# nishitbohra/RoViT-KAN-Interpretable-Vision-Transformer-for-Rose-Disease-Severity-Estimation

Measured on AMD Instinct MI355X. Metric: images/sec fwd+bwd, DeiT-Tiny+KAN 224^2, batch 256 per GPU, higher is better.
Workload: dtype bf16; 1 GPU; full RoViT-KAN (DeiT-Tiny + KAN + 3 heads) stage 4, train mode, batch 256/GPU, 224x224x3 randn images, random-init weights; step=fwd + JointLoss + bwd + grad all-reduce + clip_grad_norm(1.0) + AdamW, global_batch=256, parallelism=dp1, grad_buckets=2, rccl_world=0

## Files before the change

rovit-kan-interpretable-vision-transformer-for-rose-disease-severity-estimation_amd/csrc/gemm.hip:

```cpp
#include <cstdlib>
#include <type_traits>
#include "common.h"

#ifdef ROVIT_DEV
#define GEMM_DBG(g, bit) ((g).dbg & (bit))
#define GEMM_SET_DBG(g, v) (g).dbg = (v)
#else
#define GEMM_DBG(g, bit) (false)
#define GEMM_SET_DBG(g, v) ((void)0)
#endif

namespace {

inline bool set_max_lds(const void* fn, size_t bytes) { return rovit_set_max_lds(fn, bytes); }

constexpr int BK = 64;
constexpr int LDS_STRIDE = BK + 16;

enum { EPI_BF16 = 0, EPI_GELU = 1, EPI_RESID = 2, EPI_MUL = 3, EPI_PATCH = 4, EPI_RESID_LN = 5, EPI_LNBWD = 6,
       EPI_PATCH_IMG = 7 };

struct GemmArgs {
  const bf16* A; int lda;
  const bf16* W; int ldw;
// ... 777 lines not shown
        f32x4 o;
#pragma unroll
        for (int r = 0; r < 4; ++r) o[r] = dac[i][j][r] * gelu_grad((float)(bf16)pre[i][j][r]);
        const int row = i * 16 + l15;
        const int ch = 2 * (JT * wave + j) + (lg >> 1);
        const int phys = (ch & ~7) | ((ch & 7) ^ (row & 7));
        *(bf16x4*)(Cs + row * K + phys * 8 + 4 * (lg & 1)) = pack4(o);
      }
    barrier_lds();
    const int mbase = (tile0 + t) * BM;
#pragma unroll
    for (int q = 0; q < SMAX; ++q) {
      const int c = tid + q * NT;
      const int row = c / 24, ch = c - row * 24;
      const int m = mbase + row;
      if (m < g.M) {
        const int phys = (ch & ~7) | ((ch & 7) ^ (row & 7));
        *(bf16x8*)(g.out + (size_t)m * g.ldo + n0 + ch * 8) = *(const bf16x8*)(Cs + row * K + phys * 8);
      }
    }
    asm volatile("s_waitcnt lgkmcnt(0)" ::: "memory");
  }
}

template <int BM, int NW>
int launch_mlp_bwd(const MlpBwdArgs& g, hipStream_t st) {
  const int tiles_m = (g.M + BM - 1) / BM;
  int pmax = g_cu_budget * (768 / (NW * 64)) / g.n_tiles;
  pmax = pmax < 8 ? 8 : pmax / 8 * 8;
  const int tpw = (tiles_m + pmax - 1) / pmax;
  int P = (tiles_m + tpw - 1) / tpw;
  P = (P + 7) / 8 * 8;
  const size_t lds = (size_t)6 * BM * 192 * sizeof(bf16);
  ROVIT_CHECK_ARG(set_max_lds((const void*)mlp_bwd_dma_kernel<BM, NW>, lds), ROVIT_ERR_LAUNCH, "gemm_mlp_bwd: cannot raise the LDS limit");
  hipLaunchKernelGGL((mlp_bwd_dma_kernel<BM, NW>), dim3(P * g.n_tiles), dim3(NW * 64), lds, st, g, tpw, tiles_m);
  ROVIT_CHECK_LAUNCH("mlp_bwd_dma_kernel");
  return ROVIT_OK;
}

typedef unsigned int u32x2_t __attribute__((ext_vector_type(2)));

template <int KT, int EPI>
__global__ __launch_bounds__(768, 1) void gemm_kdma_kernel(const GemmArgs g, int tiles_per_wg, int n_tiles_m) {
  constexpr int K = 32 * KT, BM = 32, NT = 768;
  constexpr int CPRW = K / 8;
  constexpr int SLOT = BM * K;
  constexpr int PIECES = BM * CPRW / NT;
  constexpr int NSTORE = (EPI == EPI_RESID_LN) ? 7 : 6;
  constexpr int CSTR = 192 + 8;
  static_assert(BM * CPRW % NT == 0, "tile must split into whole DMA pieces");
  extern __shared__ __attribute__((aligned(16))) bf16 lds[];

  const int p = blockIdx.x;
  const int tile0 = p * tiles_per_wg;
  int ntile = n_tiles_m - tile0;
  ntile = ntile > tiles_per_wg ? tiles_per_wg : ntile;
  if (ntile <= 0) return;

  const int tid = threadIdx.x, lane = tid & 63, wave = tid >> 6;
  const int l15 = lane & 15, lg = lane >> 4;
  const bool row_wave = wave < 8;

  unsigned pk[PIECES];
#pragma unroll
  for (int i = 0; i < PIECES; ++i) {
    const int c = 64 * (wave + 12 * i) + lane;
    const int r = c / CPRW, x = c - r * CPRW;
    pk[i] = ((unsigned)r << 16) | (unsigned)(((x & ~7) | ((x & 7) ^ (r & 7))) * 8);
  }
  auto dma = [&](int tile, int slot) {
    const int row0 = tile * BM;
#pragma unroll
    for (int i = 0; i < PIECES; ++i) {
      unsigned q = pk[i];
      asm volatile("" : "+v"(q));
      int gr = row0 + (int)(q >> 16);
      gr = gr < g.M ? gr : g.M - 1;
      const bf16* src = g.A + ((unsigned)gr * (unsigned)g.lda + (q & 0xffffu));
      __builtin_amdgcn_global_load_lds((const __attribute__((address_space(1))) void*)src,
                                       (__attribute__((address_space(3))) void*)(lds + slot * SLOT + (wave + 12 * i) * 512), 16, 0, 0);
    }
  };
  dma(tile0, 0);
  if (ntile > 1) dma(tile0 + 1, 1);
  if (ntile > 2) dma(tile0 + 2, 2);

  bf16x8 wf[KT];
#pragma unroll
  for (int ks = 0; ks < KT; ++ks) wf[ks] = *(const bf16x8*)(g.W + (size_t)(16 * wave + l15) * g.ldw + ks * 32 + lg * 8);
  f32x4 bias4 = {0.f, 0.f, 0.f, 0.f};
  if (g.bias) {
    const float4 bb = *(const float4*)(g.bias + 16 * wave + 4 * lg);
    bias4 = (f32x4){bb.x, bb.y, bb.z, bb.w};
  }
  const int prow = tid >> 4, pc = tid & 15;
  wait_vmcnt<0>();

  for (int t = 0; t < ntile; ++t) {
    const int slot = t % 3;
    if (t >= 1) {
      if (t + 2 < ntile) { if (row_wave) wait_vmcnt<PIECES + NSTORE>(); else wait_vmcnt<PIECES>(); }
      else wait_vmcnt<0>();
    }
    __builtin_amdgcn_s_barrier();
    const int m = (tile0 + t) * BM + prow;
    const bool live = row_wave && m < g.M;
    const int mc = m < g.M ? m : g.M - 1;
    f32x4 xo0, xo1, xo2;
    u32x2_t hx0, hx1, hx2;
    float rr = 0.f;
    const unsigned xoff = (unsigned)mc * (unsigned)g.ldx + 4u * pc;
    float* xrow = g.xres + xoff;
    constexpr bool PREFETCH = KT <= 18;
    u32x2_t pv0, pv1, pv2;
    auto load_inputs = [&]() {
      if (EPI == EPI_LNBWD && g.xprev) {
        const bf16* prow_p = g.xprev + ((unsigned)mc * 192u + 4u * pc);
        pv0 = *(const u32x2_t*)prow_p; pv1 = *(const u32x2_t*)(prow_p + 64); pv2 = *(const u32x2_t*)(prow_p + 128);
      } else {
        xo0 = *(const f32x4*)xrow; xo1 = *(const f32x4*)(xrow + 64); xo2 = *(const f32x4*)(xrow + 128);
      }
      if (EPI == EPI_LNBWD) {
        const bf16* hrow = g.mul + ((unsigned)mc * (unsigned)g.ldm + 4u * pc);
        hx0 = *(const u32x2_t*)hrow; hx1 = *(const u32x2_t*)(hrow + 64); hx2 = *(const u32x2_t*)(hrow + 128);
        rr = g.pos[mc];
      }
    };
    if (PREFETCH && row_wave) load_inputs();
    const bool dma_now = t >= 1 && t + 2 < ntile;
    if (dma_now) dma(tile0 + t + 2, (t + 2) % 3);

    f32x4 acc[2] = {bias4, bias4};
    const bf16* Ac = lds + slot * SLOT;
#pragma unroll
    for (int ks = 0; ks < KT; ++ks) {
      const int lc = ks * 4 + lg;
#pragma unroll
      for (int i = 0; i < 2; ++i) {
        const int row = i * 16 + l15;
        const bf16x8 af = *(const bf16x8*)(Ac + row * K + ((lc & ~7) | ((lc & 7) ^ (row & 7))) * 8);
        acc[i] = mfma16(wf[ks], af, acc[i]);
      }
    }
    barrier_lds();
    bf16* Cs = lds + slot * SLOT;
#pragma unroll
    for (int i = 0; i < 2; ++i) *(bf16x4*)(Cs + (i * 16 + l15) * CSTR + 16 * wave + 4 * lg) = pack4(acc[i]);
    barrier_lds();
    if (row_wave) {
      if (!PREFETCH) load_inputs();
      float v[12];
#pragma unroll
      for (int i = 0; i < 3; ++i) {
        const bf16x4 tv = *(const bf16x4*)(Cs + prow * CSTR + 64 * i + 4 * pc);
#pragma unroll
        for (int e = 0; e < 4; ++e) v[4 * i + e] = (float)tv[e];
      }
      f32x4 xs[3] = {xo0, xo1, xo2};
      if (EPI == EPI_LNBWD && g.xprev) {
        const u32x2_t pvs[3] = {pv0, pv1, pv2};
        const bool has_in = g.tokens <= 0 || (mc % g.tokens) == 0;
#pragma unroll
        for (int i = 0; i < 3; ++i) {
          const bf16x4 pb = __builtin_bit_cast(bf16x4, pvs[i]);
          xs[i] = has_in ? (f32x4){(float)pb[0], (float)pb[1], (float)pb[2], (float)pb[3]} : (f32x4){0.f, 0.f, 0.f, 0.f};
        }
      }
      f32x4* xp = (f32x4*)(g.xres + (unsigned)mc * (unsigned)g.ldx);
      if (EPI == EPI_RESID_LN) {
        float sum = 0.f;
#pragma unroll
        for (int i = 0; i < 3; ++i) {
#pragma unroll
          for (int e = 0; e < 4; ++e) xs[i][e] += v[4 * i + e];
          sum += (xs[i][0] + xs[i][1]) + (xs[i][2] + xs[i][3]);
        }
        const float mean = wave_sum16(sum) * (1.f / 192.f);
        float qs = 0.f;
#pragma unroll
        for (int i = 0; i < 3; ++i)
#pragma unroll
          for (int e = 0; e < 4; ++e) { const float d = xs[i][e] - mean; qs += d * d; }
        const float r = rsqrtf(wave_sum16(qs) * (1.f / 192.f) + g.eps);
        if (live) {
          bf16x4* hp = (bf16x4*)(g.out + (unsigned)m * (unsigned)g.ldo);
#pragma unroll
          for (int i = 0; i < 3; ++i) xp[16 * i + pc] = xs[i];
#pragma unroll
          for (int i = 0; i < 3; ++i) {
            f32x4 tq = {(xs[i][0] - mean) * r, (xs[i][1] - mean) * r, (xs[i][2] - mean) * r, (xs[i][3] - mean) * r};
            hp[16 * i + pc] = pack4(tq);
          }
          if (pc == 0) g.rstd_out[m] = r;
        }
      } else {
        const u32x2_t hxs[3] = {hx0, hx1, hx2};
        float s1 = 0.f, s2 = 0.f;
#pragma unroll
        for (int i = 0; i < 3; ++i) {
          const bf16x4 hb = __builtin_bit_cast(bf16x4, hxs[i]);
#pragma unroll
          for (int e = 0; e < 4; ++e) { s1 += v[4 * i + e]; s2 += v[4 * i + e] * (float)hb[e]; }
        }
        const float c1 = wave_sum16(s1) * (1.f / 192.f), c2 = wave_sum16(s2) * (1.f / 192.f);
        if (live) {
          bf16x4* bp = (bf16x4*)(g.out + (unsigned)m * (unsigned)g.ldo);
#pragma unroll
          for (int i = 0; i < 3; ++i) {
            const bf16x4 hb = __builtin_bit_cast(bf16x4, hxs[i]);
#pragma unroll
            for (int e = 0; e < 4; ++e) xs[i][e] += rr * (v[4 * i + e] - c1 - (float)hb[e] * c2);
          }
          if (!g.xprev && !GEMM_DBG(g, 64)) {
#pragma unroll
            for (int i = 0; i < 3; ++i) xp[16 * i + pc] = xs[i];
          }
#pragma unroll
          for (int i = 0; i < 3; ++i) bp[16 * i + pc] = pack4(xs[i]);
        }
      }
    }
    asm volatile("s_waitcnt lgkmcnt(0)" ::: "memory");
  }
}

template <int KT, int EPI>
int launch_kdma(const GemmArgs& g0, hipStream_t st) {
  GemmArgs g = g0;
  constexpr int BM = 32;
  const int tiles_m = (g.M + BM - 1) / BM;
  int pmax = g_cu_budget;
  const int tpw = (tiles_m + pmax - 1) / pmax;
  const int P = (tiles_m + tpw - 1) / tpw;
  const size_t lds = (size_t)3 * BM * 32 * KT * sizeof(bf16);
  ROVIT_CHECK_ARG(set_max_lds((const void*)gemm_kdma_kernel<KT, EPI>, lds), ROVIT_ERR_LAUNCH, "gemm_kdma: cannot raise the LDS limit");
  hipLaunchKernelGGL((gemm_kdma_kernel<KT, EPI>), dim3(P), dim3(768), lds, st, g, tpw, tiles_m);
  ROVIT_CHECK_LAUNCH("gemm_kdma_kernel");
  return ROVIT_OK;
}
static bool kdma_enabled() { return ROVIT_KNOB(ROVIT_KNOB_KDMA, 1) != 0; }

template <int BM, int BN, int WM, int WN>
int launch_nt(const GemmArgs& g0, int epi, hipStream_t st) {
  GemmArgs g = g0;
  g.n_tiles = g.N / BN;
  const int m_tiles = (g.M + BM - 1) / BM;
  const int nwg = m_tiles * g.n_tiles;
  const size_t lds = (size_t)2 * (BM + BN) * LDS_STRIDE * sizeof(bf16);
  dim3 grid(nwg), block(WM * WN * 64);
#define LAUNCH(E)                                                                                         \
  case E: {                                                                                               \
    if (!set_max_lds((const void*)gemm_nt_kernel<BM, BN, WM, WN, E>, lds)) {                              \
      rovit_set_error("gemm_nt: cannot raise the LDS limit");                                             \
      return ROVIT_ERR_LAUNCH;                                                                            \
    }                                                                                                     \
    hipLaunchKernelGGL((gemm_nt_kernel<BM, BN, WM, WN, E>), grid, block, lds, st, g);                     \
    break;                                                                                                \
  }
  switch (epi) {
    LAUNCH(EPI_BF16) LAUNCH(EPI_GELU) LAUNCH(EPI_RESID) LAUNCH(EPI_MUL) LAUNCH(EPI_PATCH)
    default: rovit_set_error("gemm_nt: unknown epilogue %d", epi); return ROVIT_ERR_SHAPE;
  }
#undef LAUNCH
  ROVIT_CHECK_LAUNCH("gemm_nt_kernel");
  return ROVIT_OK;
}

constexpr int WG_MSTEP = 64;
constexpr int wg_stride(int t) { return ((t + 16) * 2 / 32) % 2 ? t + 16 : t + 32; }

struct WgradProb {
  const bf16* dY; int ldy;
  const bf16* A; int lda;
  int N, K;
  float* slab;
  float* colsum;
  int k_tiles, tile0;
  int a_blk, y_blk;
};
constexpr int WG_MAXPROB = 4;
struct WgradArgs {
  WgradProb p[WG_MAXPROB];
  int nprob;
  int M;
  int splits, rows_per_split, tiles_per_split;
  int patch_tokens;
  const float* img;
#ifdef ROVIT_DEV
  int dbg;
#endif
};

template <int W>
__device__ __forceinline__ void blk_map(int c, int& row, int& col) {
  if constexpr ((W / 32) % 2 == 0) {
    row = (c >> 3) % WG_MSTEP;
    col = (2 * ((c >> 3) / WG_MSTEP) + ((c >> 2) & 1)) * 32 + (c & 3) * 8;
  } else {
    row = (c >> 2) % WG_MSTEP;
    col = ((c >> 2) / WG_MSTEP) * 32 + (c & 3) * 8;
  }
}

template <int TN, int TK, bool PATCH, bool IMG = false, int WN = 2>
__global__ __launch_bounds__(128 * WN) void wgrad_kernel(const WgradArgs g) {
  constexpr int NT = 128 * WN;
  constexpr int SY = wg_stride(TN), SA = wg_stride(TK);
  constexpr int CPRY = TN / 8, CPRA = TK / 8;
  constexpr int CHY = WG_MSTEP * CPRY / NT, CHA = WG_MSTEP * CPRA / NT;
  constexpr int JN = TN / (16 * WN), IK = TK / 32;
  static_assert(TN % (16 * WN) == 0 && TK % 32 == 0 && (WG_MSTEP * CPRY) % NT == 0 && (WG_MSTEP * CPRA) % NT == 0, "tile must split evenly over the waves");
  __shared__ __attribute__((aligned(16))) bf16 lds[2 * WG_MSTEP * (SY + SA)];
  bf16* Ys = lds;
  bf16* As = lds + 2 * WG_MSTEP * SY;

  const int bid = xcd_remap(blockIdx.x, gridDim.x);
  const int split = bid / g.tiles_per_split;
  int tile = bid - split * g.tiles_per_split;
  if (split >= g.splits) return;
  int pi = 0;
#pragma unroll
  for (int j = 1; j < WG_MAXPROB; ++j)
    if (j < g.nprob && tile >= g.p[j].tile0) pi = j;
  const WgradProb pr = g.p[pi];
  tile -= pr.tile0;
  const int ntile = tile / pr.k_tiles, ktile = tile - ntile * pr.k_tiles;
  const int n0 = ntile * TN, k0 = ktile * TK;
  const int m_begin = split * g.rows_per_split;
  const int m_end = min(g.M, m_begin + g.rows_per_split);

  const int tid = threadIdx.x, lane = tid & 63, wave = tid >> 6;
  const int wk = wave / WN, wn = wave % WN;
  const int l15 = lane & 15, lg = lane >> 4;

  int y_row[CHY], y_lds[CHY], a_row[CHA], a_lds[CHA], a_col[CHA];
  const bf16* ybase[CHY];
  const bf16* abase[CHA];
  using RA = typename std::conditional<IMG, F8, bf16x8>::type;
#pragma unroll
  for (int i = 0; i < CHY; ++i) {
    const int c = tid + i * NT;
    int col;
    if (pr.y_blk) {
      blk_map<TN>(c, y_row[i], col);
      ybase[i] = pr.dY + (size_t)((n0 + col) >> 5) * g.M * 32 + ((n0 + col) & 31);
    } else {
      y_row[i] = c / CPRY;
      col = (c - y_row[i] * CPRY) * 8;
      ybase[i] = pr.dY + n0 + col;
    }
    y_lds[i] = y_row[i] * SY + col;
  }
  const int ldy_eff = pr.y_blk ? 32 : pr.ldy, lda_eff = pr.a_blk ? 32 : pr.lda;
#pragma unroll
  for (int i = 0; i < CHA; ++i) {
    const int c = tid + i * NT;
    int col;
    if (IMG) {
      const int rest = c >> 6, row_hi = rest / (CPRA / 2), pair = rest - row_hi * (CPRA / 2);
      a_row[i] = (c & 31) + 32 * row_hi;
      col = (pair * 2 + ((c >> 5) & 1)) * 8;
    } else if (pr.a_blk) {
      blk_map<TK>(c, a_row[i], col);
    } else {
      a_row[i] = c / CPRA;
      col = (c - a_row[i] * CPRA) * 8;
    }
    a_lds[i] = a_row[i] * SA + col;
    a_col[i] = k0 + col;
    abase[i] = pr.a_blk ? pr.A + (size_t)((k0 + col) >> 5) * g.M * 32 + ((k0 + col) & 31) : pr.A + k0 + col;
  }
  const int m_last = g.M - 1;
  auto load = [&](int mbase, bf16x8* ry, RA* ra) {
#pragma unroll
    for (int i = 0; i < CHY; ++i) {
      int m = mbase + y_row[i];
      m = m < m_last ? m : m_last;
      const int yr = PATCH ? m + m / (g.patch_tokens - 1) + 1 : m;
      ry[i] = *(const bf16x8*)(ybase[i] + (size_t)yr * ldy_eff);
    }
#pragma unroll
    for (int i = 0; i < CHA; ++i) {
      int m = mbase + a_row[i];
      m = m < m_last ? m : m_last;
      if constexpr (IMG) ra[i] = load_f8(patch_src(g.img, m, a_col[i]));
      else ra[i] = *(const bf16x8*)(abase[i] + (size_t)m * lda_eff);
    }
  };
  auto tobf = [&](const RA& v) -> bf16x8 {
    if constexpr (IMG) return pack8(v.lo, v.hi);
    else return v;
  };
  auto store = [&](int buf, int mbase, const bf16x8* ry, const RA* ra) {
    bf16* yd = Ys + buf * WG_MSTEP * SY;
    bf16* ad = As + buf * WG_MSTEP * SA;
    if (mbase + WG_MSTEP <= m_end) {
#pragma unroll
      for (int i = 0; i < CHY; ++i) *(bf16x8*)(yd + y_lds[i]) = ry[i];
#pragma unroll
      for (int i = 0; i < CHA; ++i) *(bf16x8*)(ad + a_lds[i]) = tobf(ra[i]);
    } else {
#pragma unroll
      for (int i = 0; i < CHY; ++i) *(bf16x8*)(yd + y_lds[i]) = keep_if(ry[i], mbase + y_row[i] < m_end);
#pragma unroll
      for (int i = 0; i < CHA; ++i) *(bf16x8*)(ad + a_lds[i]) = keep_if(tobf(ra[i]), mbase + a_row[i] < m_end);
    }
  };

  f32x4 acc[IK][JN], accb[JN];
#pragma unroll
  for (int j = 0; j < JN; ++j) {
    accb[j] = (f32x4){0.f, 0.f, 0.f, 0.f};
#pragma unroll
    for (int i = 0; i < IK; ++i) acc[i][j] = (f32x4){0.f, 0.f, 0.f, 0.f};
  }
  bf16x8 ones;
#pragma unroll
  for (int q = 0; q < 8; ++q) ones[q] = (bf16)1.0f;
  const int cs_owner = ktile * 2 + wk, cs_n = 2 * pr.k_tiles;
  bool cs_do[JN];
#pragma unroll
  for (int j = 0; j < JN; ++j) cs_do[j] = (j % cs_n) == cs_owner;

  const int nsteps = (m_end - m_begin + WG_MSTEP - 1) / WG_MSTEP;
  const bf16* Ybase = Ys + (4 * lg + (l15 >> 2)) * SY + 4 * (l15 & 3) + wn * (TN / WN);
  const bf16* Abase = As + (4 * lg + (l15 >> 2)) * SA + 4 * (l15 & 3) + wk * (TK / 2);
  auto compute = [&](int cur) {
    const bf16* Yc = Ybase + cur * WG_MSTEP * SY;
    const bf16* Ac = Abase + cur * WG_MSTEP * SA;
#pragma unroll
    for (int ms = 0; ms < WG_MSTEP / 32; ++ms) {
      bf16x8 fa[IK], fy[JN];
#pragma unroll
      for (int i = 0; i < IK; ++i) {
        const bf16* p = Ac + ms * 32 * SA + i * 16;
        fa[i] = cat4(lds_read_tr(p), lds_read_tr(p + 16 * SA));
      }
#pragma unroll
      for (int j = 0; j < JN; ++j) {
        const bf16* q = Yc + ms * 32 * SY + j * 16;
        fy[j] = cat4(lds_read_tr(q), lds_read_tr(q + 16 * SY));
      }
#pragma unroll
      for (int i = 0; i < IK; ++i)
#pragma unroll
        for (int j = 0; j < JN; ++j) acc[i][j] = mfma16(fa[i], fy[j], acc[i][j]);
#pragma unroll
      for (int j = 0; j < JN; ++j)
        if (cs_do[j]) accb[j] = mfma16(ones, fy[j], accb[j]);
    }
  };
  bf16x8 ryA[CHY], ryB[CHY];
  RA raA[CHA], raB[CHA];
  load(m_begin, ryA, raA);
  store(0, m_begin, ryA, raA);
  load(m_begin + WG_MSTEP, ryA, raA);
  load(m_begin + 2 * WG_MSTEP, ryB, raB);
  barrier_lds();
  for (int s = 0; s < nsteps; s += 2) {
    const int mb = m_begin + s * WG_MSTEP;
    if (s + 1 < nsteps) store(1, mb + WG_MSTEP, ryA, raA);
    if (!GEMM_DBG(g, 1)) load(mb + 3 * WG_MSTEP, ryA, raA);
    if (!GEMM_DBG(g, 2)) compute(0);
    barrier_lds();
    if (s + 1 < nsteps) {
      if (s + 2 < nsteps) store(0, mb + 2 * WG_MSTEP, ryB, raB);
      if (!GEMM_DBG(g, 1)) load(mb + 4 * WG_MSTEP, ryB, raB);
      if (!GEMM_DBG(g, 2)) compute(1);
      barrier_lds();
    }
  }
  float* slab = pr.slab + (size_t)split * pr.N * pr.K;
#pragma unroll
  for (int j = 0; j < JN; ++j) {
    const int n = n0 + wn * (TN / WN) + j * 16 + l15;
#pragma unroll
    for (int i = 0; i < IK; ++i) {
      const int k = k0 + wk * (TK / 2) + i * 16 + lg * 4;
      *(float4*)(slab + (size_t)n * pr.K + k) = make_float4(acc[i][j][0], acc[i][j][1], acc[i][j][2], acc[i][j][3]);
    }
    if (cs_do[j] && lg == 0) pr.colsum[(size_t)split * pr.N + n] = accb[j][0];
  }
}

struct ReduceBatch { RovitReduceDesc d[ROVIT_REDUCE_BATCH]; int first_block[ROVIT_REDUCE_BATCH + 1]; int n; };

__global__ __launch_bounds__(256) void wgrad_reduce_batch_kernel(const ReduceBatch rb) {
  __shared__ float s_pg[16][64], s_pb[16][64];
  int i = 0;
  while (i + 1 < rb.n && (int)blockIdx.x >= rb.first_block[i + 1]) ++i;
  const RovitReduceDesc& d = rb.d[i];
  const float* slab = d.ws;
  const float* colsum = d.ws + (size_t)d.splits * d.N * d.K;
  const int local = (int)blockIdx.x - rb.first_block[i];
  if (!d.gamma) {
    const int q = local * 256 + threadIdx.x;
    const int total4 = d.N * d.K / 4;
    if (q < total4) {
      const float4* sp = (const float4*)slab + q;
      float4 s = make_float4(0.f, 0.f, 0.f, 0.f);
#pragma unroll 8
      for (int j = 0; j < d.splits; ++j) {
        const float4 v = sp[(size_t)j * total4];
        s.x += v.x; s.y += v.y; s.z += v.z; s.w += v.w;
      }
      ((float4*)d.dW)[q] = s;
    }
    if (q < d.N) {
      float cb = 0.f;
#pragma unroll 8
      for (int j = 0; j < d.splits; ++j) cb += colsum[(size_t)j * d.N + q];
      d.db[q] = cb;
    }
    return;
  }
  const int kb = d.K / 64;
  const int rblk = local / kb, kblk = local - rblk * kb;
  const int r = threadIdx.x >> 4, kq = threadIdx.x & 15;
  const int n = rblk * 16 + r, k = kblk * 64 + kq * 4;
  const size_t e = (size_t)n * d.K + k;
  const size_t stride = (size_t)d.N * d.K;
  float4 G = make_float4(0.f, 0.f, 0.f, 0.f);
  float cb = 0.f;
#pragma unroll 8
  for (int j = 0; j < d.splits; ++j) {
    const float4 v = *(const float4*)(slab + (size_t)j * stride + e);
    G.x += v.x; G.y += v.y; G.z += v.z; G.w += v.w;
    cb += colsum[(size_t)j * d.N + n];
  }
  const float4 gam = *(const float4*)(d.gamma + k), bet = *(const float4*)(d.beta + k), w = *(const float4*)(d.W + e);
  *(float4*)(d.dW + e) = make_float4(fmaf(gam.x, G.x, bet.x * cb), fmaf(gam.y, G.y, bet.y * cb), fmaf(gam.z, G.z, bet.z * cb),
                                     fmaf(gam.w, G.w, bet.w * cb));
  if (kblk == 0 && kq == 0) d.db[n] = cb;
  *(float4*)&s_pg[r][kq * 4] = make_float4(w.x * G.x, w.y * G.y, w.z * G.z, w.w * G.w);
  *(float4*)&s_pb[r][kq * 4] = make_float4(w.x * cb, w.y * cb, w.z * cb, w.w * cb);
  __syncthreads();
  if (threadIdx.x < 64) {
    float sg = 0.f, sb = 0.f;
#pragma unroll
    for (int rr = 0; rr < 16; ++rr) { sg += s_pg[rr][threadIdx.x]; sb += s_pb[rr][threadIdx.x]; }
    const int slices = d.N / 16;
    float* part = d.g_scratch;
    part[(size_t)rblk * d.K + kblk * 64 + threadIdx.x] = sg;
    part[(size_t)(slices + rblk) * d.K + kblk * 64 + threadIdx.x] = sb;
  }
}

__global__ __launch_bounds__(256) void wgrad_affine_finalize_kernel(const ReduceBatch rb) {
  int i = 0;
  while (i + 1 < rb.n && (int)blockIdx.x >= rb.first_block[i + 1]) ++i;
  const RovitReduceDesc& d = rb.d[i];
  const int k = ((int)blockIdx.x - rb.first_block[i]) * 256 + threadIdx.x;
  if (k >= d.K) return;
  const float* part = d.g_scratch;
  const int slices = d.N / 16;
  float sg = 0.f, sb = 0.f;
#pragma unroll 4
  for (int sl = 0; sl < slices; ++sl) { sg += part[(size_t)sl * d.K + k]; sb += part[(size_t)(slices + sl) * d.K + k]; }
  d.dgamma[k] = sg;
  d.dbeta[k] = sb;
}

}

void rovit_set_cu_budget(int cus) { g_cu_budget = cus < 8 ? 8 : (cus > 256 ? 256 : cus); }

extern "C" int rovit_gemm_nt(const void* A, int lda, const void* W, int ldw, int M, int N, int K, const float* bias, int epi,
                             void* out, int ldo, void* out2, float* xres, int ldx, const void* mul, int ldm,
                             const float* pos, int tokens, rovit_stream_t stream) {
  ROVIT_CHECK_ARG(A && W, ROVIT_ERR_NULL, "gemm_nt: null operand");
  ROVIT_CHECK_ARG(M > 0 && N > 0 && K > 0 && K % BK == 0 && N % 96 == 0, ROVIT_ERR_SHAPE,
                  "gemm_nt: unsupported shape M=%d N=%d K=%d (K %% 64, N %% 96)", M, N, K);
  ROVIT_CHECK_ARG(lda % 8 == 0 && ldw % 8 == 0 && rovit_aligned16(A) && rovit_aligned16(W), ROVIT_ERR_ALIGN,
                  "gemm_nt: operands must be 16-byte aligned with ld %% 8 == 0");
  GemmArgs g{};
  g.A = (const bf16*)A; g.lda = lda; g.W = (const bf16*)W; g.ldw = ldw; g.M = M; g.N = N; g.K = K; g.bias = bias;
  g.out = (bf16*)out; g.ldo = ldo; g.out2 = (bf16*)out2; g.xres = xres; g.ldx = ldx; g.mul = (const bf16*)mul; g.ldm = ldm;
  g.pos = pos; g.tokens = tokens; GEMM_SET_DBG(g, ROVIT_KNOB(ROVIT_KNOB_GEMM_DBG, 0));
  const int tiled = epi & (ROVIT_GEMM_TILED_192 | ROVIT_GEMM_TILED_96);
  epi &= 0xff;
  switch (epi) {
    case EPI_BF16: case EPI_GELU: ROVIT_CHECK_ARG(out && ldo % 4 == 0, ROVIT_ERR_NULL, "gemm_nt: bf16 output missing"); break;
    case EPI_RESID: ROVIT_CHECK_ARG(xres && ldx % 4 == 0, ROVIT_ERR_NULL, "gemm_nt: residual stream missing"); break;
    case EPI_MUL: ROVIT_CHECK_ARG(out && mul, ROVIT_ERR_NULL, "gemm_nt: multiplier missing"); break;
    case EPI_PATCH: ROVIT_CHECK_ARG(xres && pos && tokens > 1 && M % (tokens - 1) == 0, ROVIT_ERR_SHAPE, "gemm_nt: bad patch epilogue"); break;
    default: ROVIT_CHECK_ARG(false, ROVIT_ERR_SHAPE, "gemm_nt: unknown epilogue %d", epi);
  }
  if (!tiled && N % 192 == 0) {
    if (K == 192 && epi == EPI_BF16) return launch_ws_dma<EPI_BF16>(g, (hipStream_t)stream);
    if (K == 192 && epi == EPI_GELU) return launch_ws_dma<EPI_GELU>(g, (hipStream_t)stream);
    if (K == 192 && epi == EPI_MUL) return launch_ws_dma<EPI_MUL>(g, (hipStream_t)stream);
    if (K == 192) return launch_ws<6, 1, 64>(g, epi, (hipStream_t)stream);
    if (K == 576) return launch_ws<9, 2, 32>(g, epi, (hipStream_t)stream);
    if (K == 768) return launch_ws<12, 2, 32>(g, epi, (hipStream_t)stream);
  }
  if (!(tiled & ROVIT_GEMM_TILED_96) && N % 192 == 0) return launch_nt<128, 192, 2, 2>(g, epi, (hipStream_t)stream);
  return launch_nt<128, 96, 2, 2>(g, epi, (hipStream_t)stream);
}

extern "C" int rovit_patch_embed_fwd(const float* images, const void* W, const float* bias, const float* pos, float* X, int batch, int tokens,
                                     rovit_stream_t stream) {
  ROVIT_CHECK_ARG(images && W && pos && X, ROVIT_ERR_NULL, "patch_embed_fwd: null pointer");
  ROVIT_CHECK_ARG(batch > 0 && tokens == 197, ROVIT_ERR_SHAPE, "patch_embed_fwd: 224x224 images in 16x16 patches (197 tokens) only");
  ROVIT_CHECK_ARG(rovit_aligned16(images) && rovit_aligned16(W) && rovit_aligned16(X) && rovit_aligned16(pos), ROVIT_ERR_ALIGN,
                  "patch_embed_fwd: buffers must be 16-byte aligned");
  GemmArgs g{};
  g.A = nullptr; g.lda = 768; g.W = (const bf16*)W; g.ldw = 768; g.M = batch * 196; g.N = 192; g.K = 768; g.bias = bias;
  g.xres = X; g.ldx = 192; g.pos = pos; g.tokens = tokens; g.img = images; GEMM_SET_DBG(g, ROVIT_KNOB(ROVIT_KNOB_GEMM_DBG, 0));
  return launch_ws<12, 2, 32>(g, EPI_PATCH_IMG, (hipStream_t)stream);
}

#ifdef ROVIT_DEV
extern "C" int rovit_gemm_mlp_bwd(const void* dY, int ldy, const void* H, int ldh, const void* W2T, const void* W1, const float* b1,
                                  int M, void* dpre, int ldo, rovit_stream_t stream) {
  ROVIT_CHECK_ARG(dY && H && W2T && W1 && b1 && dpre, ROVIT_ERR_NULL, "gemm_mlp_bwd: null pointer");
  ROVIT_CHECK_ARG(M > 0, ROVIT_ERR_SHAPE, "gemm_mlp_bwd: M must be positive");
  ROVIT_CHECK_ARG(ldy % 8 == 0 && ldh % 8 == 0 && ldo % 8 == 0 && rovit_aligned16(dY) && rovit_aligned16(H) && rovit_aligned16(W2T) &&
                      rovit_aligned16(W1) && rovit_aligned16(b1) && rovit_aligned16(dpre),
                  ROVIT_ERR_ALIGN, "gemm_mlp_bwd: operands must be 16-byte aligned with ld %% 8 == 0");
  MlpBwdArgs g{(const bf16*)dY, ldy, (const bf16*)H, ldh, (const bf16*)W2T, (const bf16*)W1, b1, (bf16*)dpre, ldo, M, 4};
  return launch_mlp_bwd<64, 12>(g, (hipStream_t)stream);
}
#endif

extern "C" size_t rovit_wgrad_workspace_bytes(int N, int K, int splits) {
  return ((size_t)splits * N * K + (size_t)splits * N) * sizeof(float);
}

static void wgrad_tile_for(int N, int K, int* tn, int* tk) {
  const int knob = ROVIT_KNOB(ROVIT_KNOB_WGRAD_TILE, 0);
  int n = knob >> 16, k = knob & 0xffff;
  if (n <= 0 || k <= 0 || N % n || K % k) { n = 96; k = 96; }
  *tn = n; *tk = k;
}

extern "C" int rovit_wgrad_splits(int M, int N, int K) {
  int tn, tk;
  wgrad_tile_for(N, K, &tn, &tk);
  const int tiles = (N / tn) * (K / tk);
  const int target = ROVIT_KNOB(ROVIT_KNOB_WGRAD_WGS, 512);
  int s = (target + tiles - 1) / tiles;
  s = (s + 7) / 8 * 8;
  const int max_s = (M + WG_MSTEP - 1) / WG_MSTEP;
  if (s > max_s) s = max_s;
  return s < 1 ? 1 : s;
}

template <int TN, int TK, int WN = 2>
static void launch_wgrad(const WgradArgs& g0, hipStream_t st) {
  WgradArgs g = g0;
  int t = 0;
  for (int j = 0; j < g.nprob; ++j) {
    g.p[j].k_tiles = g.p[j].K / TK;
    g.p[j].tile0 = t;
    t += (g.p[j].N / TN) * g.p[j].k_tiles;
  }
  g.tiles_per_split = t;
  const int nwg = g.splits * t;
  if constexpr (WN != 2) {
    hipLaunchKernelGGL((wgrad_kernel<TN, TK, false, false, WN>), dim3(nwg), dim3(128 * WN), 0, st, g);
  } else {
    if (g.patch_tokens > 0 && g.img) hipLaunchKernelGGL((wgrad_kernel<TN, TK, true, true>), dim3(nwg), dim3(256), 0, st, g);
    else if (g.patch_tokens > 0) hipLaunchKernelGGL((wgrad_kernel<TN, TK, true>), dim3(nwg), dim3(256), 0, st, g);
    else hipLaunchKernelGGL((wgrad_kernel<TN, TK, false>), dim3(nwg), dim3(256), 0, st, g);
  }
}

extern "C" int rovit_wgrad(const void* dY, int ldy, const void* A, int lda, int M, int N, int K, int splits, int patch_tokens,
                           float* ws, rovit_stream_t stream) {
  ROVIT_CHECK_ARG(dY && A && ws, ROVIT_ERR_NULL, "wgrad: null pointer");
  ROVIT_CHECK_ARG(M > 0 && N % 96 == 0 && K % 96 == 0 && splits > 0, ROVIT_ERR_SHAPE, "wgrad: unsupported shape N=%d K=%d", N, K);
  ROVIT_CHECK_ARG(ldy % 8 == 0 && lda % 8 == 0 && rovit_aligned16(dY) && rovit_aligned16(A), ROVIT_ERR_ALIGN, "wgrad: alignment");
  WgradArgs g{};
  g.nprob = 1;
  g.p[0] = WgradProb{(const bf16*)dY, ldy, (const bf16*)A, lda, N, K, ws, ws + (size_t)splits * N * K, 0, 0};
  g.M = M;
  g.splits = splits;
  g.rows_per_split = ((M + splits - 1) / splits + WG_MSTEP - 1) / WG_MSTEP * WG_MSTEP;
  g.patch_tokens = patch_tokens;
  GEMM_SET_DBG(g, ROVIT_KNOB(ROVIT_KNOB_GEMM_DBG, 0) >> 4);
  int tn, tk;
  wgrad_tile_for(N, K, &tn, &tk);
  hipStream_t st = (hipStream_t)stream;
  switch ((tn << 16) | tk) {
    case (96 << 16) | 96: launch_wgrad<96, 96>(g, st); break;
#ifdef ROVIT_DEV
    case (64 << 16) | 96: launch_wgrad<64, 96>(g, st); break;
    case (96 << 16) | 64: launch_wgrad<96, 64>(g, st); break;
    case (64 << 16) | 64: launch_wgrad<64, 64>(g, st); break;
    case (96 << 16) | 192: launch_wgrad<96, 192>(g, st); break;
    case (192 << 16) | 96: launch_wgrad<192, 96>(g, st); break;
#endif
    default: rovit_set_error("wgrad: no kernel for tile %d x %d", tn, tk); return ROVIT_ERR_SHAPE;
  }
  ROVIT_CHECK_LAUNCH("wgrad_kernel");
  return ROVIT_OK;
}

extern "C" int rovit_patch_embed_wgrad(const void* dY, int ldy, const float* images, int batch, int tokens, int N, int splits, float* ws,
                                       rovit_stream_t stream) {
  ROVIT_CHECK_ARG(dY && images && ws, ROVIT_ERR_NULL, "patch_embed_wgrad: null pointer");
  ROVIT_CHECK_ARG(batch > 0 && tokens == 197 && N % 96 == 0 && splits > 0, ROVIT_ERR_SHAPE, "patch_embed_wgrad: unsupported shape");
  ROVIT_CHECK_ARG(ldy % 8 == 0 && rovit_aligned16(dY) && rovit_aligned16(images), ROVIT_ERR_ALIGN, "patch_embed_wgrad: alignment");
  const int M = batch * (tokens - 1), K = 768;
  WgradArgs g{};
  g.nprob = 1;
  g.p[0] = WgradProb{(const bf16*)dY, ldy, nullptr, K, N, K, ws, ws + (size_t)splits * N * K, 0, 0};
  g.M = M;
  g.splits = splits;
  g.rows_per_split = ((M + splits - 1) / splits + WG_MSTEP - 1) / WG_MSTEP * WG_MSTEP;
  g.patch_tokens = tokens;
  g.img = images;
  GEMM_SET_DBG(g, ROVIT_KNOB(ROVIT_KNOB_GEMM_DBG, 0) >> 4);
  if (N % 192 == 0) launch_wgrad<192, 96>(g, (hipStream_t)stream);
  else launch_wgrad<96, 96>(g, (hipStream_t)stream);
  ROVIT_CHECK_LAUNCH("wgrad_kernel (patch, image gather)");
  return ROVIT_OK;
}

int rovit_wgrad_batch(const RovitWgradDesc* descs, int n, int M, int splits, rovit_stream_t stream) {
  ROVIT_CHECK_ARG(descs && n >= 1 && n <= WG_MAXPROB && M > 0 && splits > 0, ROVIT_ERR_SHAPE, "wgrad_batch: bad arguments");
  WgradArgs g{};
  g.nprob = n;
  for (int j = 0; j < n; ++j) {
    const RovitWgradDesc& d = descs[j];
    ROVIT_CHECK_ARG(d.dY && d.A && d.ws, ROVIT_ERR_NULL, "wgrad_batch: null pointer");
    ROVIT_CHECK_ARG(d.N % 96 == 0 && d.K % 192 == 0, ROVIT_ERR_SHAPE, "wgrad_batch: unsupported shape N=%d K=%d", d.N, d.K);
    ROVIT_CHECK_ARG(d.ldy % 8 == 0 && d.lda % 8 == 0 && rovit_aligned16(d.dY) && rovit_aligned16(d.A), ROVIT_ERR_ALIGN, "wgrad_batch: alignment");
    ROVIT_CHECK_ARG(!(d.a_blk && d.K % 32) && !(d.y_blk && d.N % 32), ROVIT_ERR_SHAPE, "wgrad_batch: chunk-major operands need 32-column chunks");
    g.p[j] = WgradProb{(const bf16*)d.dY, d.ldy, (const bf16*)d.A, d.lda, d.N, d.K, d.ws, d.ws + (size_t)splits * d.N * d.K, 0, 0, d.a_blk, d.y_blk};
  }
  g.M = M;
  g.splits = splits;
  g.rows_per_split = ((M + splits - 1) / splits + WG_MSTEP - 1) / WG_MSTEP * WG_MSTEP;
  GEMM_SET_DBG(g, ROVIT_KNOB(ROVIT_KNOB_GEMM_DBG, 0) >> 4);
  if (n == 1 && g.p[0].K % 96 == 0) launch_wgrad<96, 96>(g, (hipStream_t)stream);
  else {
    for (int j = 0; j < n; ++j) ROVIT_CHECK_ARG(descs[j].N % 192 == 0 && descs[j].K % 192 == 0, ROVIT_ERR_SHAPE, "wgrad_batch: N, K %% 192 for 192-wide tiles");
    launch_wgrad<192, 192, 4>(g, (hipStream_t)stream);
  }
  ROVIT_CHECK_LAUNCH("wgrad_kernel (batch)");
  return ROVIT_OK;
}

extern "C" int rovit_wgrad_multi(const void* const* dY, const int* ldy, const void* const* A, const int* lda, const int* N, const int* K,
                                 float* const* ws, int n, int M, int splits, rovit_stream_t stream) {
  ROVIT_CHECK_ARG(dY && ldy && A && lda && N && K && ws && n >= 1 && n <= WG_MAXPROB, ROVIT_ERR_NULL, "wgrad_multi: bad arguments");
  RovitWgradDesc d[WG_MAXPROB];
  for (int j = 0; j < n; ++j) d[j] = {dY[j], ldy[j], A[j], lda[j], N[j], K[j], ws[j]};
  return rovit_wgrad_batch(d, n, M, splits, stream);
}

extern "C" int rovit_wgrad_multi_ex(const void* const* dY, const int* ldy, const void* const* A, const int* lda, const int* N, const int* K,
                                    float* const* ws, const int* a_blk, const int* y_blk, int n, int M, int splits, rovit_stream_t stream) {
  ROVIT_CHECK_ARG(dY && ldy && A && lda && N && K && ws && n >= 1 && n <= WG_MAXPROB, ROVIT_ERR_NULL, "wgrad_multi_ex: bad arguments");
  RovitWgradDesc d[WG_MAXPROB];
  for (int j = 0; j < n; ++j) d[j] = {dY[j], ldy[j], A[j], lda[j], N[j], K[j], ws[j], a_blk ? a_blk[j] : 0, y_blk ? y_blk[j] : 0};
  return rovit_wgrad_batch(d, n, M, splits, stream);
}

extern "C" int rovit_wgrad_reduce(const float* ws, int splits, int N, int K, const float* gamma, const float* beta,
                                  const float* W, float* dW, float* db, float* dgamma, float* dbeta, float* g_scratch,
                                  rovit_stream_t stream) {
  const RovitReduceDesc d{ws, splits, N, K, gamma, beta, W, dW, db, dgamma, dbeta, g_scratch};
  return rovit_wgrad_reduce_batch(&d, 1, stream);
}

int rovit_wgrad_reduce_batch(const RovitReduceDesc* descs, int n, rovit_stream_t stream) {
#ifdef ROVIT_DEV
  if (ROVIT_KNOB(ROVIT_KNOB_SKIP_WGRAD_REDUCE, 0)) return ROVIT_OK;
#endif
  ROVIT_CHECK_ARG(descs && n > 0 && n <= ROVIT_REDUCE_BATCH, ROVIT_ERR_SHAPE, "wgrad_reduce_batch: bad batch size %d", n);
  ReduceBatch rb{}, ab{};
  int blocks = 0, fblocks = 0;
  for (int i = 0; i < n; ++i) {
    const RovitReduceDesc& d = descs[i];
    ROVIT_CHECK_ARG(d.ws && d.dW && d.db, ROVIT_ERR_NULL, "wgrad_reduce_batch: null pointer");
    rb.d[i] = d;
    rb.first_block[i] = blocks;
    if (d.gamma) {
      ROVIT_CHECK_ARG(d.beta && d.W && d.dgamma && d.dbeta && d.g_scratch, ROVIT_ERR_NULL, "wgrad_reduce_batch: affine un-fold needs beta/W/outputs");
      ROVIT_CHECK_ARG(d.N % 16 == 0 && d.K % 64 == 0 && 2 * (d.N / 16) <= d.N, ROVIT_ERR_SHAPE, "wgrad_reduce_batch: affine un-fold needs N %% 16 == 0, K %% 64 == 0");
      blocks += (d.N / 16) * (d.K / 64);
      ab.d[ab.n] = d;
      ab.first_block[ab.n] = fblocks;
      fblocks += (d.K + 255) / 256;
      ab.n++;
    } else {
      const int nthreads = d.N * d.K / 4 > d.N ? d.N * d.K / 4 : d.N;
      blocks += (nthreads + 255) / 256;
    }
  }
  rb.n = n; rb.first_block[n] = blocks;
  ab.first_block[ab.n] = fblocks;
  hipLaunchKernelGGL(wgrad_reduce_batch_kernel, dim3(blocks), dim3(256), 0, (hipStream_t)stream, rb);
  ROVIT_CHECK_LAUNCH("wgrad_reduce_batch_kernel");
  if (ab.n > 0) {
    hipLaunchKernelGGL(wgrad_affine_finalize_kernel, dim3(fblocks), dim3(256), 0, (hipStream_t)stream, ab);
    ROVIT_CHECK_LAUNCH("wgrad_affine_finalize_kernel");
  }
  return ROVIT_OK;
}

extern "C" int rovit_gemm_resid_ln(const void* A, int lda, const void* W, int ldw, int M, int K, const float* bias, float* X,
                                   void* xhat_out, float* rstd_out, float eps, rovit_stream_t stream) {
  ROVIT_CHECK_ARG(A && W && X, ROVIT_ERR_NULL, "gemm_resid_ln: null pointer");
  ROVIT_CHECK_ARG(M > 0 && (K == 192 || K == 576 || K == 768), ROVIT_ERR_SHAPE, "gemm_resid_ln: K must be 192/576/768 (got %d)", K);
  ROVIT_CHECK_ARG(lda % 8 == 0 && ldw % 8 == 0 && rovit_aligned16(A) && rovit_aligned16(W) && rovit_aligned16(X), ROVIT_ERR_ALIGN,
                  "gemm_resid_ln: alignment");
  ROVIT_CHECK_ARG(!xhat_out || rstd_out, ROVIT_ERR_NULL, "gemm_resid_ln: rstd_out missing");
  GemmArgs g{};
  g.A = (const bf16*)A; g.lda = lda; g.W = (const bf16*)W; g.ldw = ldw; g.M = M; g.N = 192; g.K = K; g.bias = bias;
  g.xres = X; g.ldx = 192; g.out = (bf16*)xhat_out; g.ldo = 192; g.rstd_out = rstd_out; g.eps = eps; GEMM_SET_DBG(g, ROVIT_KNOB(ROVIT_KNOB_GEMM_DBG, 0));
  if (K == 192) return launch_ws<6, 1, 64>(g, EPI_RESID_LN, (hipStream_t)stream);
  if (kdma_enabled() && xhat_out && K == 576) return launch_kdma<18, EPI_RESID_LN>(g, (hipStream_t)stream);
  if (K == 576) return launch_ws<9, 2, 32>(g, EPI_RESID_LN, (hipStream_t)stream);
  return launch_ws<12, 2, 32>(g, EPI_RESID_LN, (hipStream_t)stream);
}

static int gemm_ln_bwd_impl(const void* dY, int ldy, const void* W, int ldw, int M, int K, const void* xhat, const float* rstd,
                            float* dX, const void* dXb_in, int cls_step, void* dXb, rovit_stream_t stream);
extern "C" int rovit_gemm_ln_bwd(const void* dY, int ldy, const void* W, int ldw, int M, int K, const void* xhat, const float* rstd,
                                 float* dX, const void* dXb_in, void* dXb, rovit_stream_t stream) {
  return gemm_ln_bwd_impl(dY, ldy, W, ldw, M, K, xhat, rstd, dX, dXb_in, 0, dXb, stream);
}
int rovit_gemm_ln_bwd_cls(const void* dY, int ldy, const void* W, int ldw, int M, int K, const void* xhat, const float* rstd,
                          const void* dXb_in, int cls_step, void* dXb, rovit_stream_t stream) {
  ROVIT_CHECK_ARG(dXb_in && cls_step > 0, ROVIT_ERR_NULL, "gemm_ln_bwd_cls: needs the bf16 incoming gradient and a row step");
  return gemm_ln_bwd_impl(dY, ldy, W, ldw, M, K, xhat, rstd, nullptr, dXb_in, cls_step, dXb, stream);
}
static int gemm_ln_bwd_impl(const void* dY, int ldy, const void* W, int ldw, int M, int K, const void* xhat, const float* rstd,
                            float* dX, const void* dXb_in, int cls_step, void* dXb, rovit_stream_t stream) {
  ROVIT_CHECK_ARG(dY && W && xhat && rstd && (dX || dXb_in) && dXb, ROVIT_ERR_NULL, "gemm_ln_bwd: null pointer");
  ROVIT_CHECK_ARG(rovit_aligned16(dXb_in) && rovit_aligned16(dXb), ROVIT_ERR_ALIGN, "gemm_ln_bwd: alignment");
  ROVIT_CHECK_ARG(M > 0 && (K == 192 || K == 576 || K == 768), ROVIT_ERR_SHAPE, "gemm_ln_bwd: K must be 192/576/768 (got %d)", K);
  ROVIT_CHECK_ARG(ldy % 8 == 0 && ldw % 8 == 0 && rovit_aligned16(dY) && rovit_aligned16(W) && rovit_aligned16(dX), ROVIT_ERR_ALIGN,
                  "gemm_ln_bwd: alignment");
  GemmArgs g{};
  g.A = (const bf16*)dY; g.lda = ldy; g.W = (const bf16*)W; g.ldw = ldw; g.M = M; g.N = 192; g.K = K;
  g.mul = (const bf16*)xhat; g.ldm = 192; g.pos = rstd; g.xres = dX; g.ldx = 192; g.out = (bf16*)dXb; g.ldo = 192; g.xprev = (const bf16*)dXb_in; g.tokens = cls_step; GEMM_SET_DBG(g, ROVIT_KNOB(ROVIT_KNOB_GEMM_DBG, 0) | (ROVIT_KNOB(ROVIT_KNOB_SKIP_DX_FP32_STORE, 0) ? 64 : 0));
  if (K == 192) return launch_ws<6, 1, 64>(g, EPI_LNBWD, (hipStream_t)stream);
  if (kdma_enabled() && K == 576) return launch_kdma<18, EPI_LNBWD>(g, (hipStream_t)stream);
  if (K == 576) return launch_ws<9, 2, 32>(g, EPI_LNBWD, (hipStream_t)stream);
  return launch_ws<12, 2, 32>(g, EPI_LNBWD, (hipStream_t)stream);
}
```

Before: 63070 images/sec.

## Use a four-stage direct-to-LDS ring pipeline for the batched 192x192 wgrad kernel

Adds a new body for the eight-wave 192x192 weight-gradient kernel. It streams 32-row slabs of dY and A straight from global memory into a four-deep LDS ring with global_load_lds, and reads MFMA fragments with transposing ds_read_b64_tr_b16 in hand-written asm. The aim is to drop the register-staged load/store double buffer and keep more loads in flight, so that global latency hides behind MFMA work. In exchange it needs dynamic LDS above the default limit, an extra launch check, and stride/M limits for the 32-bit offset arithmetic.

```diff
diff --git a/rovit-kan-interpretable-vision-transformer-for-rose-disease-severity-estimation_amd/csrc/gemm.hip b/rovit-kan-interpretable-vision-transformer-for-rose-disease-severity-estimation_amd/csrc/gemm.hip
--- a/rovit-kan-interpretable-vision-transformer-for-rose-disease-severity-estimation_amd/csrc/gemm.hip
+++ b/rovit-kan-interpretable-vision-transformer-for-rose-disease-severity-estimation_amd/csrc/gemm.hip
@@ -1103,8 +1103,8 @@
   }
 }
 
-template <int TN, int TK, bool PATCH, bool IMG = false, int WN = 2>
-__global__ __launch_bounds__(128 * WN) void wgrad_kernel(const WgradArgs g) {
+template <int TN, int TK, bool PATCH, bool IMG, int WN>
+__device__ __forceinline__ void wgrad_regs_body(const WgradArgs& g) {
   constexpr int NT = 128 * WN;
   constexpr int SY = wg_stride(TN), SA = wg_stride(TK);
   constexpr int CPRY = TN / 8, CPRA = TK / 8;
@@ -1282,6 +1282,197 @@
     }
     if (cs_do[j] && lg == 0) pr.colsum[(size_t)split * pr.N + n] = accb[j][0];
   }
+}
+
+constexpr int WG_RSTEP = 32, WG_RING = 4;
+
+template <int TN, int TK, int WN>
+__device__ __forceinline__ void wgrad_ring_body(const WgradArgs& g) {
+  constexpr int NW = 2 * WN, RS = WG_RSTEP, RING = WG_RING;
+  constexpr int YB = TN / 16, AB = TK / 16;
+  constexpr int PIECES = (YB + AB) / NW;
+  constexpr int STAGE = RS * (TN + TK);
+  constexpr int JN = TN / (16 * WN), IK = TK / 32;
+  static_assert(TN % 64 == 0 && TK % 64 == 0 && (YB + AB) % NW == 0 && TN % (16 * WN) == 0 && RING >= 3 && RING <= 4, "ring tile");
+  extern __shared__ __attribute__((aligned(16))) bf16 lds[];
+
+  const int bid = xcd_remap(blockIdx.x, gridDim.x);
+  const int split = bid / g.tiles_per_split;
+  int tile = bid - split * g.tiles_per_split;
+  if (split >= g.splits) return;
+  int pi = 0;
+#pragma unroll
+  for (int j = 1; j < WG_MAXPROB; ++j)
+    if (j < g.nprob && tile >= g.p[j].tile0) pi = j;
+  const WgradProb pr = g.p[pi];
+  tile -= pr.tile0;
+  const int ntile = tile / pr.k_tiles, ktile = tile - ntile * pr.k_tiles;
+  const int n0 = ntile * TN, k0 = ktile * TK;
+  const int m_begin = split * g.rows_per_split;
+  const int m_end = min(g.M, m_begin + g.rows_per_split);
+  const int nsteps = (m_end - m_begin + RS - 1) / RS;
+
+  const int tid = threadIdx.x, lane = tid & 63, wave = __builtin_amdgcn_readfirstlane(tid >> 6);
+  const int wk = wave / WN, wn = wave % WN;
+  const int l15 = lane & 15, lg = lane >> 4;
+
+  const bf16* pbase[PIECES];
+  int pld[PIECES];
+  unsigned poff[PIECES];
+  const int prow = lane >> 3;
+#pragma unroll
+  for (int i = 0; i < PIECES; ++i) {
+    const int b = wave + NW * i;
+    const bool is_a = b >= YB;
+    const int bb = is_a ? b - YB : b;
+    const int row = 8 * (bb & 3) + prow, q = lane & 7;
+    const int col = (bb >> 2) * 64 + ((((q >> 1) ^ (row >> 1)) & 3) << 4) + (q & 1) * 8;
+    const bf16* P = is_a ? pr.A : pr.dY;
+    const int c0 = is_a ? k0 : n0, ld = is_a ? pr.lda : pr.ldy;
+    if (is_a ? pr.a_blk : pr.y_blk) {
+      pbase[i] = P + (size_t)(c0 >> 5) * g.M * 32;
+      pld[i] = 32;
+      poff[i] = 2u * ((unsigned)(col >> 5) * (unsigned)g.M * 32u + (unsigned)(row * 32 + (col & 31)));
+    } else {
+      pbase[i] = P + c0;
+      pld[i] = ld;
+      poff[i] = 2u * ((unsigned)row * (unsigned)ld + (unsigned)col);
+    }
+  }
+  const int m_last = g.M - 1;
+  auto issue = [&](int t, int stage) {
+    const int mb = m_begin + t * RS;
+    const bool full = mb + RS <= m_end;
+#pragma unroll
+    for (int i = 0; i < PIECES; ++i) {
+      const int b = wave + NW * i;
+      unsigned off = poff[i];
+      asm volatile("" : "+v"(off));
+      if (!full) {
+        const int over = mb + 8 * (((b >= YB ? b - YB : b)) & 3) + prow - m_last;
+        if (over > 0) off -= 2u * (unsigned)over * (unsigned)pld[i];
+      }
+      const char* src = (const char*)(pbase[i] + (size_t)mb * pld[i]) + off;
+      __builtin_amdgcn_global_load_lds((const __attribute__((address_space(1))) void*)src,
+                                       (__attribute__((address_space(3))) void*)(lds + stage * STAGE + b * 512), 16, 0, 0);
+    }
+  };
+
+  f32x4 acc[IK][JN], accb[JN];
+#pragma unroll
+  for (int j = 0; j < JN; ++j) {
+    accb[j] = (f32x4){0.f, 0.f, 0.f, 0.f};
+#pragma unroll
+    for (int i = 0; i < IK; ++i) acc[i][j] = (f32x4){0.f, 0.f, 0.f, 0.f};
+  }
+  bf16x8 ones;
+#pragma unroll
+  for (int q = 0; q < 8; ++q) ones[q] = (bf16)1.0f;
+  const int cs_owner = ktile * 2 + wk, cs_n = 2 * pr.k_tiles;
+  bool cs_do[JN];
+#pragma unroll
+  for (int j = 0; j < JN; ++j) cs_do[j] = (j % cs_n) == cs_owner;
+
+  const int fr = 4 * lg + (l15 >> 2), key = (fr >> 1) & 3;
+  const unsigned lds0 = (unsigned)(size_t)((__attribute__((address_space(3))) bf16*)lds);
+  unsigned aaddr[IK], yaddr[JN];
+#pragma unroll
+  for (int i = 0; i < IK; ++i) {
+    const int c = wk * (TK / 2) + i * 16;
+    aaddr[i] = lds0 + 2u * (unsigned)(RS * TN + (c >> 6) * (RS * 64) + fr * 64 + ((((c >> 4) & 3) ^ key) << 4) + 4 * (l15 & 3));
+  }
+#pragma unroll
+  for (int j = 0; j < JN; ++j) {
+    const int c = wn * (TN / WN) + j * 16;
+    yaddr[j] = lds0 + 2u * (unsigned)((c >> 6) * (RS * 64) + fr * 64 + ((((c >> 4) & 3) ^ key) << 4) + 4 * (l15 & 3));
+  }
+  auto compute = [&](int t, int stage) {
+    constexpr int O0 = 0, O1 = 16 * 64 * 2;
+    static_assert(IK == 6 && JN == 3, "the fragment-read block is written for the 192 x 192 eight-wave tile");
+    unsigned aa[IK], ya[JN];
+#pragma unroll
+    for (int i = 0; i < IK; ++i) aa[i] = aaddr[i] + (unsigned)(stage * STAGE * 2);
+#pragma unroll
+    for (int j = 0; j < JN; ++j) ya[j] = yaddr[j] + (unsigned)(stage * STAGE * 2);
+    bf16x4 al[IK], ah[IK], yl[JN], yh[JN];
+    asm volatile(
+        "ds_read_b64_tr_b16 %0, %18 offset:%27\n\tds_read_b64_tr_b16 %6, %18 offset:%28\n\t"
+        "ds_read_b64_tr_b16 %12, %24 offset:%27\n\tds_read_b64_tr_b16 %15, %24 offset:%28\n\t"
+        "ds_read_b64_tr_b16 %13, %25 offset:%27\n\tds_read_b64_tr_b16 %16, %25 offset:%28\n\t"
+        "ds_read_b64_tr_b16 %14, %26 offset:%27\n\tds_read_b64_tr_b16 %17, %26 offset:%28\n\t"
+        "ds_read_b64_tr_b16 %1, %19 offset:%27\n\tds_read_b64_tr_b16 %7, %19 offset:%28\n\t"
+        "ds_read_b64_tr_b16 %2, %20 offset:%27\n\tds_read_b64_tr_b16 %8, %20 offset:%28\n\t"
+        "ds_read_b64_tr_b16 %3, %21 offset:%27\n\tds_read_b64_tr_b16 %9, %21 offset:%28\n\t"
+        "ds_read_b64_tr_b16 %4, %22 offset:%27\n\tds_read_b64_tr_b16 %10, %22 offset:%28\n\t"
+        "ds_read_b64_tr_b16 %5, %23 offset:%27\n\tds_read_b64_tr_b16 %11, %23 offset:%28\n\t"
+        "s_waitcnt lgkmcnt(0)"
+        : "=&v"(al[0]), "=&v"(al[1]), "=&v"(al[2]), "=&v"(al[3]), "=&v"(al[4]), "=&v"(al[5]),
+          "=&v"(ah[0]), "=&v"(ah[1]), "=&v"(ah[2]), "=&v"(ah[3]), "=&v"(ah[4]), "=&v"(ah[5]),
+          "=&v"(yl[0]), "=&v"(yl[1]), "=&v"(yl[2]), "=&v"(yh[0]), "=&v"(yh[1]), "=&v"(yh[2])
+        : "v"(aa[0]), "v"(aa[1]), "v"(aa[2]), "v"(aa[3]), "v"(aa[4]), "v"(aa[5]), "v"(ya[0]), "v"(ya[1]), "v"(ya[2]), "n"(O0), "n"(O1)
+        : "memory");
+    bf16x8 fa[IK], fy[JN];
+#pragma unroll
+    for (int i = 0; i < IK; ++i) fa[i] = cat4(al[i], ah[i]);
+#pragma unroll
+    for (int j = 0; j < JN; ++j) fy[j] = cat4(yl[j], yh[j]);
+    const int rem = m_end - (m_begin + t * RS);
+    if (rem < RS) {
+      u32x4 keep;
+#pragma unroll
+      for (int d = 0; d < 4; ++d) {
+        const int r0 = 16 * (d >> 1) + 4 * lg + 2 * (d & 1);
+        keep[d] = (r0 < rem ? 0xffffu : 0u) | (r0 + 1 < rem ? 0xffff0000u : 0u);
+      }
+#pragma unroll
+      for (int j = 0; j < JN; ++j) fy[j] = __builtin_bit_cast(bf16x8, __builtin_bit_cast(u32x4, fy[j]) & keep);
+    }
+#pragma unroll
+    for (int i = 0; i < IK; ++i)
+#pragma unroll
+      for (int j = 0; j < JN; ++j) acc[i][j] = mfma16(fa[i], fy[j], acc[i][j]);
+#pragma unroll
+    for (int j = 0; j < JN; ++j)
+      if (cs_do[j]) accb[j] = mfma16(ones, fy[j], accb[j]);
+  };
+#pragma unroll
+  for (int t = 0; t < RING - 1; ++t)
+    if (t < nsteps) issue(t, t);
+  for (int t = 0, stage = 0; t < nsteps; ++t) {
+    const int ahead = nsteps - 1 - t;
+    if (ahead >= RING - 2) wait_vmcnt<PIECES * (RING - 2)>();
+    else if (ahead == 1) wait_vmcnt<PIECES>();
+    else wait_vmcnt<0>();
+    asm volatile("s_waitcnt lgkmcnt(0)" ::: "memory");
+    __builtin_amdgcn_s_barrier();
+    asm volatile("" ::: "memory");
+    const int prev = stage == 0 ? RING - 1 : stage - 1;
+    if (t + RING - 1 < nsteps) issue(t + RING - 1, prev);
+    compute(t, stage);
+    stage = stage == RING - 1 ? 0 : stage + 1;
+  }
+  float* slab = pr.slab + (size_t)split * pr.N * pr.K;
+#pragma unroll
+  for (int j = 0; j < JN; ++j) {
+    const int n = n0 + wn * (TN / WN) + j * 16 + l15;
+#pragma unroll
+    for (int i = 0; i < IK; ++i) {
+      const int k = k0 + wk * (TK / 2) + i * 16 + lg * 4;
+      *(float4*)(slab + (size_t)n * pr.K + k) = make_float4(acc[i][j][0], acc[i][j][1], acc[i][j][2], acc[i][j][3]);
+    }
+    if (cs_do[j] && lg == 0) pr.colsum[(size_t)split * pr.N + n] = accb[j][0];
+  }
+}
+
+template <int TN, int TK, bool PATCH, int WN>
+constexpr bool wgrad_uses_ring() { return !PATCH && WN == 4 && TN % 64 == 0 && TK % 64 == 0; }
+template <int TN, int TK>
+constexpr size_t wgrad_ring_lds_bytes() { return (size_t)WG_RING * WG_RSTEP * (TN + TK) * sizeof(bf16); }
+
+template <int TN, int TK, bool PATCH, bool IMG = false, int WN = 2>
+__global__ __launch_bounds__(128 * WN) void wgrad_kernel(const WgradArgs g) {
+  if constexpr (wgrad_uses_ring<TN, TK, PATCH, WN>()) wgrad_ring_body<TN, TK, WN>(g);
+  else wgrad_regs_body<TN, TK, PATCH, IMG, WN>(g);
 }
 
 struct ReduceBatch { RovitReduceDesc d[ROVIT_REDUCE_BATCH]; int first_block[ROVIT_REDUCE_BATCH + 1]; int n; };
@@ -1448,7 +1639,7 @@
 }
 
 template <int TN, int TK, int WN = 2>
-static void launch_wgrad(const WgradArgs& g0, hipStream_t st) {
+static bool launch_wgrad(const WgradArgs& g0, hipStream_t st) {
   WgradArgs g = g0;
   int t = 0;
   for (int j = 0; j < g.nprob; ++j) {
@@ -1459,12 +1650,15 @@
   g.tiles_per_split = t;
   const int nwg = g.splits * t;
   if constexpr (WN != 2) {
-    hipLaunchKernelGGL((wgrad_kernel<TN, TK, false, false, WN>), dim3(nwg), dim3(128 * WN), 0, st, g);
+    constexpr size_t lds = wgrad_uses_ring<TN, TK, false, WN>() ? wgrad_ring_lds_bytes<TN, TK>() : 0;
+    if (lds && !set_max_lds((const void*)wgrad_kernel<TN, TK, false, false, WN>, lds)) return false;
+    hipLaunchKernelGGL((wgrad_kernel<TN, TK, false, false, WN>), dim3(nwg), dim3(128 * WN), lds, st, g);
   } else {
     if (g.patch_tokens > 0 && g.img) hipLaunchKernelGGL((wgrad_kernel<TN, TK, true, true>), dim3(nwg), dim3(256), 0, st, g);
     else if (g.patch_tokens > 0) hipLaunchKernelGGL((wgrad_kernel<TN, TK, true>), dim3(nwg), dim3(256), 0, st, g);
     else hipLaunchKernelGGL((wgrad_kernel<TN, TK, false>), dim3(nwg), dim3(256), 0, st, g);
   }
+  return true;
 }
 
 extern "C" int rovit_wgrad(const void* dY, int ldy, const void* A, int lda, int M, int N, int K, int splits, int patch_tokens,
@@ -1538,7 +1732,9 @@
   if (n == 1 && g.p[0].K % 96 == 0) launch_wgrad<96, 96>(g, (hipStream_t)stream);
   else {
     for (int j = 0; j < n; ++j) ROVIT_CHECK_ARG(descs[j].N % 192 == 0 && descs[j].K % 192 == 0, ROVIT_ERR_SHAPE, "wgrad_batch: N, K %% 192 for 192-wide tiles");
-    launch_wgrad<192, 192, 4>(g, (hipStream_t)stream);
+    for (int j = 0; j < n; ++j)
+      ROVIT_CHECK_ARG(descs[j].ldy < (1 << 24) && descs[j].lda < (1 << 24) && M < (1 << 22), ROVIT_ERR_SHAPE, "wgrad_batch: row stride or M too large");
+    ROVIT_CHECK_ARG((launch_wgrad<192, 192, 4>(g, (hipStream_t)stream)), ROVIT_ERR_LAUNCH, "wgrad_batch: cannot raise the LDS limit");
   }
   ROVIT_CHECK_LAUNCH("wgrad_kernel (batch)");
   return ROVIT_OK;
```

Result: no change. 63490 images/sec (median of 6 runs) (+0.7%).
